# kai422/DAS3R

Hardware: AMD Instinct MI355X
Metric: render fwd+bwd Msplats/s at 1080p (higher is better)
Workload: dtype f32; 1 GPU; 1M random splats, 1920x1080, SH degree 3, forward+backward (BASELINE.json configs[3], constant P); splats_per_gpu=1000000, splats_per_gpu_final=1000000, init_steps=30, sh_degree=3, num_rendered=2614506, api=GaussianRasterizer.forward + autograd backward (drop-in surface), parallelism=1 independent scenes, one per GPU

## Files before the change

das3r_amd/csrc/api.hip:

```cpp
#include <stdarg.h>
#include <string.h>

#include <vector>

#include "common.h"
#include <algorithm>

namespace das3r {

static thread_local char g_err[512] = "";

void set_error(const char *fmt, ...) {
    va_list ap;
    va_start(ap, fmt);
    vsnprintf(g_err, sizeof(g_err), fmt, ap);
    va_end(ap);
}

struct ProfRec {
    const char *name;
    hipEvent_t start, stop;
};
static bool g_prof_on = false;
static std::vector<ProfRec> g_prof;
// ... 53 lines not shown
            const char *pp = strchr(e, 'p');
            w.render_bwd_pix = pp ? atoi(pp + 1) : 0;
            const char *po = strchr(e, 'o');
            w.render_bwd_occ = po ? atoi(po + 1) : 5;
        }
        if (w.render_bwd == 7) {
            const char *d = e;
            while (*d && (*d < '0' || *d > '9')) d++;
            w.render_bwd_mb = *d ? atoi(d) : 128;
            w.render_bwd_pix = strchr(e, 'q') ? 9 : (strchr(e, 's') ? 8 : 0);
        }
        if (w.render_bwd == 3) {
            const char *d = e;
            while (*d && (*d < '0' || *d > '9')) d++;
            w.render_bwd_mb = (*d ? atoi(d) : 256) + (strncmp(e, "scana", 5) == 0 ? 1000 : 0);
        }
    }
    if ((e = env("DAS3R_BWD_REDUCE"))) { w.bwd_reduce_set = true; w.bwd_reduce_shfl = e[0] == 's'; }
    w.tickets = -1;
    if ((e = env("DAS3R_TICKETS"))) w.tickets = e[0] == 'a' ? 0 : (e[0] == 'n' ? 1 << 30 : ((e[0] >= '1' && e[0] <= '9') ? atoi(e) : -1));
    w.deterministic = (e = env("DAS3R_DETERMINISTIC")) && e[0] != '0';
    w.bwd_buckets = -1;
    if ((e = env("DAS3R_BWD_BUCKETS"))) w.bwd_buckets = atoi(e);
    w.tile_strip = 8;
    w.tile_chunk = -1;
    if ((e = env("DAS3R_TILE_CHUNK"))) { const int v = atoi(e); w.tile_chunk = (v >= 0 && v <= 64 && (v & (v - 1)) == 0) ? v : -1; }
    if ((e = env("DAS3R_TILE_STRIP"))) w.tile_strip = std::max(0, std::min(63, atoi(e)));
    w.inject_fault = g_inject_fault;
    w.mutate = g_mutate;
    g_sw = w;
    __atomic_store_n(&g_sw_loaded, true, __ATOMIC_RELEASE);
}
const Switches &switches() {
    if (!__atomic_load_n(&g_sw_loaded, __ATOMIC_ACQUIRE)) load_switches();
    return g_sw;
}

constexpr int MAX_DEVICES = 64;
static int g_threads_on_device[MAX_DEVICES] = {};
struct ThreadRegistrar {
    bool on[MAX_DEVICES] = {};
    void add(int dev) {
        if (!on[dev]) { on[dev] = true; __atomic_fetch_add(&g_threads_on_device[dev], 1, __ATOMIC_RELAXED); }
    }
    ~ThreadRegistrar() {
        for (int d = 0; d < MAX_DEVICES; d++)
// ... 107 lines not shown
    L->g_dhist = take(4 * 256);
    L->g_ghist = take(4 * 4 * RADIX_SIZE);
    L->g_ticket = take(256);
    L->g_status = take(onesweep_status_bytes((int64_t)Pn, 4));
    L->g_scan_status = take(scan_status_bytes((int)Pn));
    L->g_ctrl_bytes = o - L->g_ghist;
    if (shjac) L->g_shjac = take(4 * 9 * Pn);
    L->pub.geom_bytes = o;
    o = 0;
    L->b_keyA = take(4 * In);
    L->b_keyB = take(4 * In);
    L->b_valA = take(4 * In);
    L->b_valB = take(4 * In);
    L->b_hist = take(4 * (size_t)RADIX_SIZE * (size_t)(L->chunksI > 0 ? L->chunksI : 1));
    L->b_totals = take(4 * RADIX_SIZE);
    L->b_gid_of = take(4 * In);
    L->b_slot = take(4 * In);
    L->b_e2 = take(4 * In);
    L->b_ghist = take(4 * 4 * RADIX_SIZE);
    L->b_ticket = take(256);
    L->b_status = take(onesweep_status_bytes((int64_t)In, L->tile_passes + 1));
    L->b_ctrl_bytes = o - L->b_ghist;
    L->b_ckpt = take(((size_t)In / BUCKET + (size_t)(L->ntiles > 0 ? L->ntiles : 1) + 2) * 256 * 16);
    L->pub.binning_bytes = o;
    const size_t npix_d = (size_t)W * (size_t)H;
    L->d_ckpt = take(((size_t)In / BUCKET + (size_t)(L->ntiles > 0 ? L->ntiles : 1) + 2) * 256 * 16);
    L->d_recs = take(16 * SPLAT_REC * Pn);
    L->d_dpix = take(4 * 3 * (npix_d > 0 ? npix_d : 1));
    L->d_bg = take(16);
    L->d_dz = take(4 * Pn);
    L->d_bytes = o;
    L->pub.point_list = (L->tile_passes & 1) ? L->b_valB : L->b_valA;
    o = 0;
    const size_t npix = (size_t)W * (size_t)H;
    L->pub.final_T = take(4 * (npix > 0 ? npix : 1));
    L->pub.n_contrib = take(4 * (npix > 0 ? npix : 1));
    L->pub.ranges = take(8 * (size_t)(L->ntiles > 0 ? L->ntiles : 1));
    L->i_order = take(4 * (size_t)(L->ntiles > 0 ? L->ntiles : 1));
    L->pub.img_bytes = o;
}

static bool dhist_slots(hipStream_t s, uint32_t **use, uint32_t **next) {
    struct Slot { int dev; hipStream_t stream; uint32_t *buf; uint32_t turn; };
    static thread_local std::vector<Slot> slots;
    int dev = 0;
    if (hipGetDevice(&dev) != hipSuccess) return false;
// ... 361 lines not shown
            verdict.longest = (uint32_t)longest;
            const uint32_t crowd16 = mb->host[15];
            verdict.fine = (longest > mean + (mean * 4) / 5 && longest >= 4096) || crowd16 >= CROWDED16;
            if (switches().verbose) fprintf(stderr, "[das3r] tile lists: longest %lld, mean %lld, %.1f of 64 consecutive entries in one quadrant -> %s kernels\n", (long long)longest,
                                            (long long)mean, crowd16 / 16.0, verdict.fine ? "2x2-region" : "block");
        }
        lb.prefer_regions = verdict.fine;
        lb.tile_order = nullptr;
        if (verdict.fine && cap > 0 && use_quad_lanes(L, lb) && L.ntiles <= 1024 && !switches().tile_lpt_off && (switches().render_fwd == 0 || switches().render_fwd == 5)) {
            if ((r = launch_tile_lpt(saved->img, L, (uint32_t)cap, a->debug != 0, s))) return r;
            lb.tile_order = (const uint32_t *)(saved->img + L.i_order);
        }
        if (verdict.fine && cap > 0 && use_quad_lanes(L, lb)) {
            const uint32_t hint = std::min<uint32_t>(63u, verdict.longest / (uint32_t)BUCKET + 2u);
            saved->flags |= 1u | (hint << 8);
        }
        if (local_order && cap > 0) {
            lb.point_list = (uint32_t *)(saved->binning + L.pub.point_list);
            lb.slot_list = (uint32_t *)(saved->binning + L.b_slot);
            lb.keys = dead_keys;
            lb.host_flag = mb->dev + 10;
        }
        if ((r = join.now())) return r;
        return launch_render_forward(a, in->colors_precomp, out->out_color, saved->geom, saved->binning, saved->img, L, lb, s, out->out_invdepth,
                                     depth ? (float4 *)(saved->binning + L.d_ckpt) : nullptr);
    };
    auto prefiltered_ok = [&]() -> int {
        if (!a->prefiltered || mb->host[12] != count_tag) return DAS3R_OK;
        set_error("Point is filtered although prefiltered is set. This shouldn't happen!");
        return DAS3R_ERR_INVALID_ARG;
    };
    int64_t I, cap;
    if ((local || seg) && verdict.last_I >= 0 && a->capacity_hint != -1 && !switches().capacity_exact) {
        cap = std::max(verdict.last_I + verdict.last_I / 4, verdict.peak_I + verdict.peak_I / 20) + 4096;
        if (cap > (int64_t)0x7FFFFF00) cap = (int64_t)0x7FFFFF00;
        compute_layout(P, cap, W, H, &L, shjac);
        apply_seg();
        saved->binning = alloc_binning(user, depth ? L.d_bytes : L.pub.binning_bytes);
        if (!saved->binning) { set_error("scratch allocation failed (binning %zu B)", L.pub.binning_bytes); return DAS3R_ERR_ALLOC; }
        char *&emit_ring = T->emit_ring;
        bool &emit_ring_dirty = T->emit_ring_dirty;
        uint32_t &emit_last_tag = T->emit_last_tag;
        constexpr size_t EMIT_SLOT_BYTES = sizeof(uint32_t) * EMIT_SLOT_WORDS + sizeof(unsigned long long) * EMIT_STATUS_GRANULES;
        const bool fused_emit = local && grid_is_resident(div_up(P, 256)) && !switches().fused_emit_off;
        uint32_t *emit_slot = nullptr;
        if (fused_emit) {
// ... 385 lines not shown
```

das3r_amd/csrc/common.h:

```cpp
#pragma once
#include <hip/hip_runtime.h>
#include <stdint.h>
#include <stdio.h>

#include "../../include/das3r_raster.h"
#include "pretransform_math.h"

#define TILE_X 16
#define TILE_Y 16
#define TILE_PIX 256
#define WAVE 64
#define NEAR_PLANE 0.001f

namespace das3r {

void set_error(const char *fmt, ...);

struct Switches {
    int sort_ipl;
    bool sort_classic;
    bool rect_upstream;
    bool verbose;
    int binning;
    bool capacity_exact;
    bool fused_emit_off;
    bool no_sh_stage;
    int render_fwd;
    int render_bwd;
    int render_bwd_mb;
    int tile_chunk;
    int scan_items;
    bool deterministic;
    int render_bwd_occ;
    bool tile_lpt_off;
    int render_bwd_pix;
    bool bwd_reduce_set, bwd_reduce_shfl;
    bool ablate_set;
    int ablate;
    int tickets;
    int bwd_pad_lds, fwd_pad_lds;
    int bwd_buckets;
    int inject_fault;
    int mutate;
    bool fwd_no_prefetch;
    int split_colour;
    int tile_strip;
};
const Switches &switches();

#define HIP_TRY(expr)                                                                          \
    do {                                                                                       \
        hipError_t _e = (expr);                                                                \
        if (_e != hipSuccess) {                                                                \
            das3r::set_error("%s failed: %s (%s:%d)", #expr, hipGetErrorString(_e), __FILE__, __LINE__); \
            return DAS3R_ERR_HIP;                                                              \
        }                                                                                      \
    } while (0)

#define KERNEL_CHECK(stream, debug, name)                                                      \
    do {                                                                                       \
        hipError_t _e = hipGetLastError();                                                     \
        if (_e == hipSuccess && (debug)) _e = hipStreamSynchronize(stream);                    \
        if (_e != hipSuccess) {                                                                \
            das3r::set_error("kernel %s failed: %s", name, hipGetErrorString(_e));             \
            return DAS3R_ERR_HIP;                                                              \
        }                                                                                      \
    } while (0)

// ... 77 lines not shown
int sort_ipl_override();
static inline int sort_items_per_lane(int64_t n) {
    const int o = sort_ipl_override();
    return o ? o : (n >= (int64_t)(1 << 21) ? 16 : (n >= (1 << 17) ? 8 : 4));
}
static inline int sort_num_chunks(int64_t n) { return n == 0 ? 0 : div_up(n, (int64_t)WAVE * sort_items_per_lane(n)); }
__host__ __device__ static inline int tile_digit_width(int tbits) {
    const int passes = (tbits + 7) / 8;
    return passes > 0 ? (tbits + passes - 1) / passes : 8;
}
static inline int tile_bits(int ntiles) {
    int b = 0;
    while ((1 << b) < ntiles) b++;
    return b < 1 ? 1 : b;
}

constexpr int BUCKET = 1024;
constexpr int SPLAT_REC = 4;

constexpr uint32_t DEPTH_SAVED_FLAG = 2u;
constexpr uint32_t SHJAC_SAVED_FLAG = 4u;
constexpr uint32_t NO_BACKWARD_IN_FLAG = 8u;
constexpr uint32_t ANTIALIAS_FLAG = 16u;
struct Layout {
    das3r_raster_layout pub;
    size_t g_keyA, g_keyB, g_valA, g_valB, g_hist, g_totals, g_blocksums, g_count, g_off_by_gid, g_rect;
    size_t b_keyA, b_keyB, b_valA, b_valB, b_hist, b_totals, b_gid_of, b_slot;
    size_t b_e2;
    size_t b_ckpt;
    size_t d_ckpt, d_recs, d_dpix, d_bg, d_dz, d_bytes;
    size_t g_ghist, g_ticket, g_status, g_scan_status, g_ctrl_bytes;
    int64_t capacity;
    size_t b_ghist, b_ticket, b_status, b_ctrl_bytes;
    int tiles_x, tiles_y, ntiles, tbits, tile_passes;
    int chunksP, chunksI;
    int dbits, kbits, kshift;
    int part_passes;
    size_t g_dhist;
    size_t g_shjac;
    const uint32_t *dhist_ptr;
    size_t i_order;
};
static inline int seg_dbits(const Layout &L, int passes) { return 8 * (passes < 3 ? passes : 3) - L.tbits; }

struct LocalBin {
    float4 *ckpt;
    uint32_t *point_list, *slot_list;
    uint32_t *keys;
    uint32_t *host_flag;
    uint32_t flag_value;
    uint32_t last_g, cap;
    bool prefer_regions;
// ... 19 lines not shown
struct SideStream {
    hipStream_t stream;
    hipEvent_t fork, join;
    int colour_blocks;
};
int launch_preprocess(const das3r_raster_args *a, const das3r_raster_in *in, int32_t *radii, char *geom, char *img, char *binning_ctrl,
                      size_t binning_ctrl_bytes, const Layout &L, unsigned long long *arrive, uint32_t *host_out, uint32_t tag,
                      hipStream_t s, const EmitArgs *emit, uint32_t *dhist, uint32_t *dhist_next, bool aa ,
                      const SideStream *side = nullptr);
int launch_sh_colour(const das3r_raster_args *a, const das3r_raster_in *in, char *geom, const Layout &L, const SideStream *side);
int launch_mark_visible(int P, const float *means3D, const float *viewmatrix, uint8_t *present, hipStream_t s);
int launch_depth_sort(int P, char *geom, const Layout &L, int part, char *binning_ctrl, size_t binning_ctrl_bytes, bool debug, hipStream_t s);
int launch_scan(int P, char *geom, const Layout &L, uint32_t *host_out, uint32_t tag, bool debug, hipStream_t s, bool index_order = false);
int launch_scan_emit(int P, int64_t cap, const int32_t *radii, char *geom, char *binning, const Layout &L, uint32_t *host_out, uint32_t tag,
                     bool debug, hipStream_t s, bool index_order = false);
size_t scan_status_bytes(int P);
int launch_binning_scan_emit(int P, int64_t I, const int32_t *radii, char *geom, char *binning, const Layout &L, bool ctrl_zeroed,
                             uint32_t *host_out, uint32_t tag, bool debug, hipStream_t s, bool index_order = false);
size_t onesweep_status_bytes(int64_t n, int passes);
int launch_onesweep_depth_sort(int P, char *geom, const Layout &L, int part, uint32_t *zero_ptr, uint32_t zero_words, bool debug,
                               hipStream_t s);
int launch_onesweep_partition(int64_t cap, char *geom, char *binning, const Layout &L, uint32_t **keys_final, bool debug, hipStream_t s,
                              uint32_t *ghist_override = nullptr, uint32_t *err_override = nullptr);
bool use_row_private(int64_t instances, int ntiles);
bool use_quad_lanes(const Layout &L, const LocalBin &lb);
inline PreXform pre_xform(const das3r_raster_in *in) {
    PreXform x = {nullptr, nullptr, nullptr, nullptr, nullptr, nullptr, nullptr, nullptr, nullptr};
    if (in && in->pre) {
        const das3r_pretransform *p = in->pre;
        x = PreXform{p->xyz, p->rot, p->scaling, p->opacity_raw, p->conf_flat, p->mask_index, p->R, p->t, p->Lq};
    }
    return x;
}
int launch_render_forward_regions(const das3r_raster_args *a, float *out_color, char *geom, char *binning, char *img, const Layout &L, const LocalBin &lb,
                                  hipStream_t s, float *out_invdepth, float4 *dckpt);
int launch_tile_lpt(char *img, const Layout &L, uint32_t cap, bool debug, hipStream_t s);
int launch_list_skew(const char *img, const char *binning, const char *geom, const Layout &L, uint32_t cap, uint32_t last_g, uint32_t *mailbox_words, uint32_t tag,
                     bool debug, hipStream_t s);
int launch_render_forward_slices(const das3r_raster_args *a, float *out_color, char *geom, char *binning, char *img, const Layout &L, const LocalBin &lb,
                                 hipStream_t s);
int launch_render_forward_lanes(const das3r_raster_args *a, float *out_color, char *geom, char *binning, char *img, const Layout &L,
                                const LocalBin &lb, hipStream_t s, float *out_invdepth, float4 *dckpt);
int launch_render_forward_rows(const das3r_raster_args *a, float *out_color, char *geom, char *binning, char *img, const Layout &L,
                               const LocalBin &lb, hipStream_t s, float *out_invdepth, float4 *dckpt);
int launch_render_backward_mfma(const das3r_raster_args *a, const float *dL_dpix, char *geom, char *binning, char *img, const Layout &L,
                                float *partial, hipStream_t s);
size_t stream_scratch_bytes(int64_t capacity);
int launch_render_backward_stream(const das3r_raster_args *a, const float *dL_dpix, char *geom, char *binning, char *img, const Layout &L,
                                  float *scratch, hipStream_t s);
int launch_render_backward_scan(const das3r_raster_args *a, const float *dL_dpix, char *geom, char *binning, char *img, const Layout &L,
                                float *partial, int mb, int slices, hipStream_t s);
int launch_render_backward_blk(const das3r_raster_args *a, const float *dL_dpix, char *geom, char *binning, char *img, const Layout &L,
                               float *partial, int mb, int slices, hipStream_t s);
int launch_render_backward_regions(const das3r_raster_args *a, const float *dL_dpix, char *geom, char *binning, char *img, const Layout &L,
                               float *partial, int mb, int slices, hipStream_t s);
constexpr int LOCAL_MAX = 1024;
bool grid_is_resident(int nblocks);
bool use_onesweep();
bool use_tight_rect();
int launch_binning(int P, int64_t I, int W, int H, const int32_t *radii, char *geom, char *binning, char *img, const Layout &L,
                   bool fused_scan, uint32_t *host_late, uint32_t tag, bool debug, hipStream_t s, uint32_t **dead_keys = nullptr,
                   uint32_t *emit_slot = nullptr ,
                   uint32_t *seg_host_flag = nullptr, uint32_t seg_flag_value = 0 );
int launch_segment_sort(int64_t cap, const uint32_t *n_ptr, const uint32_t *keys_final, int fbits, uint32_t *point_list, uint32_t *slot_list,
                        const uint32_t *depth_key, uint32_t last_g, uint32_t *scratch_keys, uint32_t *host_flag, uint32_t flag_value, bool debug,
                        hipStream_t s, int dbits, uint2 *ranges, const uint32_t *err, uint32_t *host_late, uint32_t tag, uint32_t inject);
int launch_render_forward(const das3r_raster_args *a, const float *colors_precomp, float *out_color, char *geom, char *binning,
                          char *img, const Layout &L, const LocalBin &lb, hipStream_t s, float *out_invdepth ,
                          float4 *dckpt );
int launch_depth_pass_inputs(int P, int npix, const char *geom, const Layout &L, char *binning, const float *dL_dinvdepth, hipStream_t s, bool debug);
int launch_depth_fold(int P, const char *geom, const Layout &L, float *partial, const float *partial_depth, float *dz, hipStream_t s, bool debug);
int launch_render_backward(const das3r_raster_args *a, const float *dL_dpix, char *geom, char *binning, char *img, const Layout &L,
                           float *partial, hipStream_t s, bool *quad_rows, int64_t num_rendered, uint32_t fwd_flags );
int launch_render_aux_forward(int P, int W, int H, int C, const float *feat, float *out, const char *geom, const char *binning, const char *img,
                              const Layout &L, int64_t num_rendered, bool debug, hipStream_t s);
int launch_render_aux_adjoint(int P, int W, int H, int C, const float *dL_dout, float *dL_dfeat, int accumulate, float *partial, const char *geom,
// ... 39 lines not shown
```

das3r_amd/csrc/render_bwd.hip:

```cpp
#include "render_common.h"

namespace das3r {

constexpr int NACC = 9;

template <bool USE_DPP>
__global__ void __launch_bounds__(256) render_backward_kernel(
    const uint2 *__restrict__ ranges, const uint32_t *__restrict__ point_list, int W, int H, int tiles_x, int ntiles_strip ,
    const float4 *__restrict__ xyh, const float4 *__restrict__ conic_opacity, const float4 *__restrict__ rgbd,
    const float *__restrict__ bg, const float *__restrict__ final_T, const uint32_t *__restrict__ n_contrib,
    const float *__restrict__ dL_dpix, const uint32_t *__restrict__ slot_list, float *__restrict__ partial , int ablate,
    uint32_t last_g, uint32_t cap ,
    unsigned long long *__restrict__ pairs ) {
    __shared__ StagedSplat stage[TILE_PIX];
    __shared__ uint32_t s_slot[TILE_PIX];
    __shared__ float acc[TILE_PIX * NACC];
    __shared__ uint32_t s_max[4];

    const int ntiles = packed_ntiles(ntiles_strip);
    const int tile = xcd_tile(blockIdx.x, ntiles_strip, tiles_x);
    if (tile < 0) return;
    const int tid = threadIdx.x, lane = __lane_id(), wave = tid >> 6;
    const int bx = tile % tiles_x, by = tile / tiles_x;
    int px, py;
// ... 131 lines not shown
        if (sw.deterministic && kind == 1) {
            kind = 6;
            mb = 64;
        }
    }
#ifdef DAS3R_EXPERIMENTS
    if (kind == 5) {
        *quad_rows = true;
        return launch_render_backward_stream(a, dL_dpix, geom, binning, img, L, partial, s);
    }
    if (kind == 2) return launch_render_backward_mfma(a, dL_dpix, geom, binning, img, L, partial, s);
#else
    if (kind == 5 || kind == 2) {
        set_error("DAS3R_RENDER_BWD=%s: this library was built without the superseded kernels (make EXPERIMENTS=1)", kind == 5 ? "stream" : "mfma");
        return DAS3R_ERR_INVALID_ARG;
    }
#endif
    if (kind == 3 || kind == 6 || kind == 7) {
        int slices = sw.bwd_buckets;
        if (slices < 0) slices = (int)std::min<int64_t>(32, std::max<int64_t>(1, num_rendered / ((int64_t)BUCKET * std::max(L.ntiles, 1))));
        if (slices > 1 && mb > 256) slices = 1;
        const int hint = (int)((fwd_flags >> 8) & 0xFFu);
        if (sw.bwd_buckets < 0 && kind == 7 && slices > 1 && hint > slices) slices = std::min(hint, 64);
        if (kind == 6) return launch_render_backward_blk(a, dL_dpix, geom, binning, img, L, partial, mb, slices, s);
        if (kind == 7) return launch_render_backward_regions(a, dL_dpix, geom, binning, img, L, partial, mb, slices, s);
        return launch_render_backward_scan(a, dL_dpix, geom, binning, img, L, partial, mb, slices, s);
    }
    const bool use_dpp = !sw.bwd_reduce_shfl;
    const int ablate = sw.ablate;
#define ARGS                                                                                                                 \
    (const uint2 *)(img + L.pub.ranges), (const uint32_t *)(binning + L.pub.point_list), a->image_width, a->image_height,    \
        L.tiles_x, pack_tiles(L), (const float4 *)(geom + L.pub.xy), (const float4 *)(geom + L.pub.conic_opacity),                \
        (const float4 *)(geom + L.pub.rgbd), a->bg, (const float *)(img + L.pub.final_T),                                    \
        (const uint32_t *)(img + L.pub.n_contrib), dL_dpix, (const uint32_t *)(binning + L.b_slot), partial, ablate, \
        (uint32_t)(a->P - 1), (uint32_t)L.capacity, pair_counters()
    const int pad_lds = sw.bwd_pad_lds;
    if (use_dpp) DAS3R_LAUNCH((render_backward_kernel<true>), dim3(xcd_grid(L)), dim3(TILE_PIX), pad_lds, s, ARGS);
    else DAS3R_LAUNCH((render_backward_kernel<false>), dim3(xcd_grid(L)), dim3(TILE_PIX), 0, s, ARGS);
#undef ARGS
    KERNEL_CHECK(s, a->debug, "render_backward");
    return DAS3R_OK;
}

}
```

das3r_amd/csrc/render_bwd_blk.hip:

```cpp
#include "render_blk.h"

namespace das3r {

template <int MB, int PIX, int ABL = 0, int OCC = 5, bool LAST = false>
__global__ void __launch_bounds__(256, OCC) render_backward_blk_kernel(
    const uint2 *__restrict__ ranges, const uint32_t *__restrict__ point_list, int W, int H, int tiles_x, int ntiles_strip ,
    const float4 *__restrict__ xyh, const float4 *__restrict__ conic_opacity, const float4 *__restrict__ rgbd,
    const float *__restrict__ bg, const float *__restrict__ final_T, const uint32_t *__restrict__ n_contrib,
    const float *__restrict__ dL_dpix, const uint32_t *__restrict__ slot_list, float *__restrict__ partial ,
    uint32_t last_g, uint32_t cap ,
    const float4 *__restrict__ ckpt ,
    unsigned long long *__restrict__ pairs_arg ) {
#ifdef DAS3R_EXPERIMENTS
    DECODE_PAIRS_OR_TRACE(pairs_arg)
#else
    unsigned long long *const pairs = pairs_arg;
#endif
    static_assert(MB >= 64 && MB <= 256 && MB % 8 == 0, "entries per round (one-byte list entries)");
    constexpr int LIST_STRIDE = MB + 4;
    constexpr int OFF_STAGE = 0;
    constexpr int OFF_ACC = OFF_STAGE + MB * (int)sizeof(StagedSplat);
    constexpr int OFF_ACC1 = OFF_ACC + 4 * MB * 8 * 4;
    constexpr int OFF_SLOT = OFF_ACC1 + 4 * MB * 4;
    constexpr int OFF_LIST = OFF_SLOT + MB * 4;
    constexpr int OFF_MAX = OFF_LIST + 16 * LIST_STRIDE;
    constexpr int OFF_CST = OFF_MAX + 16;
    constexpr int OFF_ST = OFF_CST + (PIX > 0 ? 16 * PIX_CST_ROW : 0);
    constexpr int LDS_BYTES = OFF_ST + (PIX == 2 ? 16 * PIX_ST_ROW : 0);
    __shared__ __attribute__((aligned(16))) char lds[LDS_BYTES];
    StagedSplat *const stage = reinterpret_cast<StagedSplat *>(lds + OFF_STAGE);
    float *const acc8 = reinterpret_cast<float *>(lds + OFF_ACC);
    float *const acc1 = reinterpret_cast<float *>(lds + OFF_ACC1);
    uint32_t *const s_slot = reinterpret_cast<uint32_t *>(lds + OFF_SLOT);
    uint32_t *const s_max = reinterpret_cast<uint32_t *>(lds + OFF_MAX);

// ... 66 lines not shown
            for (uint32_t f = tid; f < ntail; f += TILE_PIX) {
                const uint32_t t = f / NACC, q = f - t * NACC;
                partial[(size_t)min(slot_list[range.x + lo + max_contrib + t], cap - 1u) * NACC + q] = 0.f;
            }
        }
        PHASE_MARK(14)
        if (max_contrib == 0u) continue;
        if (slices > 1) {
            float T0 = my_T_final, R0 = 0.f;
            if (bk < nbuckets - 1) {
                const int cpix = (ppy - by * TILE_Y) * 16 + (ppx - bx * TILE_X);
                const float4 far = ckpt_slot(const_cast<float4 *>(ckpt), range, tile, bk)[cpix];
                const float4 fin = ckpt_slot(const_cast<float4 *>(ckpt), range, tile, nbuckets - 1)[cpix];
                T0 = far.x;
                R0 = px.d0 * (fin.y - far.y) + px.d1 * (fin.z - far.z) + px.d2 * (fin.w - far.w);
            }
            px.T = T0;
            px.R = R0 + my_tfbg;
            if constexpr (PIX == 2) {
                *reinterpret_cast<float2 *>(st_row + s * 8) = make_float2(px.T, px.R);
                __builtin_amdgcn_fence(__ATOMIC_ACQ_REL, "workgroup");
            }
        }
        uint32_t g_ahead = 0u, slot_ahead = 0u;
        if (tid < min(MB, (int)max_contrib)) {
            const uint32_t pos = range.x + lo + max_contrib - 1 - tid;
            g_ahead = point_list[pos];
            slot_ahead = slot_list[pos];
        }
        for (int i = 0; i < rounds; i++) {
            const int done_before = i * MB;
            const int n = min(MB, (int)max_contrib - done_before);
            if (tid < n) {
                const uint32_t g = min(g_ahead, last_g);
                s_slot[tid] = min(slot_ahead, cap - 1u);
                stage[tid].xyh = xyh[(size_t)g * SPLAT_REC];
                stage[tid].co = conic_opacity[(size_t)g * SPLAT_REC];
                stage[tid].rgbd = rgbd[(size_t)g * SPLAT_REC];
            }
            if (i + 1 < rounds && tid < min(MB, (int)max_contrib - done_before - MB)) {
                const uint32_t pos = range.x + lo + max_contrib - 1 - (done_before + MB) - tid;
                g_ahead = point_list[pos];
                slot_ahead = slot_list[pos];
            }
            {
                const long long base = (long long)lo + (long long)max_contrib - done_before - MB;
                const long long rel = (long long)last_contributor - base;
                px.lastrel = (float)(rel < 0 ? 0ll : (rel > MB ? (long long)MB : rel));
                if constexpr (PIX > 0) *reinterpret_cast<float *>(cst_row + s * 16 + 12) = px.lastrel;
            }
            float blk_last[4] = {0.f, 0.f, 0.f, 0.f};
            if constexpr (LAST) {
                int v = (int)px.lastrel;
#pragma unroll
                for (int o = 8; o >= 1; o >>= 1) v = max(v, __shfl_xor(v, o, 64));
#pragma unroll
                for (int r = 0; r < 4; r++) blk_last[r] = (float)__builtin_amdgcn_readlane(v, 16 * r);
            }
            __syncthreads();
            PHASE_MARK(9)

            int len[4] = {0, 0, 0, 0};
#pragma unroll
            for (int k = 0; k < (MB + 63) / 64; k++) {
                const int j = k * 64 + lane;
                const int jc = j < n ? j : 0;
                const float4 p = stage[jc].xyh;
                const float4 co = stage[jc].co;
                const bool qhit = (j < n) && ((ABL & 16) ? rect_hit_tight_tau(p, co, splat_tau(co.w), (float)qx0, (float)qy0) : true);
                float hd1, hd2;
                diagonal_extents(p, co, hd1, hd2);
                const float posrel_j = (float)(MB - 1 - j);
#pragma unroll
                for (int r = 0; r < 4; r++) {
                    const bool hit = qhit && (!LAST || posrel_j < blk_last[r]) && block_hit_oct(p.x, p.y, p.z, p.w, (ABL & 8) ? 1e30f : hd1, (ABL & 8) ? 1e30f : hd2,
                                                           (float)(qx0 + ((r & 1) << 2)) + 1.5f, (float)(qy0 + ((r >> 1) << 2)) + 1.5f);
                    const uint64_t m = __ballot(hit);
                    const int at = len[r] + (int)__builtin_amdgcn_mbcnt_hi((uint32_t)(m >> 32), __builtin_amdgcn_mbcnt_lo((uint32_t)m, 0u));
                    if (hit) wave_lists[r * LIST_STRIDE + at] = (uint8_t)j;
                    len[r] += __popcll(m);
                }
            }
            const int my_len = row == 0 ? len[0] : (row == 1 ? len[1] : (row == 2 ? len[2] : len[3]));
            const int longest = (ABL & 1) ? 0 : __builtin_amdgcn_readfirstlane(max(max(len[0], len[1]), max(len[2], len[3])));
            __builtin_amdgcn_fence(__ATOMIC_ACQ_REL, "workgroup");
            PHASE_MARK(10)

            v4f p_lo4 = {0.f, 0.f, 0.f, 0.f}, p_hi4 = p_lo4;
            float p_syy = 0.f;
            float *p_rec8 = acc8, *p_rec1 = acc1;
            bool p_valid = false;
            auto add_pass = [&](const int r) {
                if (row == r && p_valid && !(ABL & 2)) {
                    const v4f o0 = *reinterpret_cast<const v4f *>(p_rec8), o1 = *reinterpret_cast<const v4f *>(p_rec8 + 4 * MB * 4);
                    const float o2 = *p_rec1;
                    *reinterpret_cast<v4f *>(p_rec8) = o0 + p_lo4;
                    *reinterpret_cast<v4f *>(p_rec8 + 4 * MB * 4) = o1 + p_hi4;
                    *p_rec1 = o2 + p_syy;
                }
                __builtin_amdgcn_fence(__ATOMIC_ACQ_REL, "wavefront");
            };
            batches_done += (longest + 15) >> 4;
            for (int b = 0; b < longest; b += 16) {
// ... 59 lines not shown
                    store_partial_row(rowp, a[0], a[1], a[2], (Sgx * co.x + Sgy * co.y) * (float)W ,
                                      (Sgy * co.z + Sgx * co.y) * (float)H, kh * a[6], kh * a[7], kh * a[8], a[3]);
                }
            }
            PHASE_MARK(13)
        }
    }
    PHASE_END(8)
#ifdef DAS3R_EXPERIMENTS
    BLK_STAMP(trace, 5, 1)
    if (trace != nullptr) {
        asm volatile("s_waitcnt vmcnt(0)" ::: "memory");
        BLK_STAMP(trace, 5, 2)
        if (threadIdx.x == 0 && blockIdx.x < (uint32_t)TRACE_WGS) trace[((size_t)5 * TRACE_WGS + blockIdx.x) * TRACE_STAMPS + 3] = range.y - range.x;
    }
#endif
    if (pairs != nullptr && lane == 0 && batches_done > 0) {
        atomicAdd(pairs + 1, (unsigned long long)batches_done * 1024ull);
        atomicAdd(pairs + 3, (unsigned long long)batches_done * 16ull);
    }
}

int launch_render_backward_blk(const das3r_raster_args *a, const float *dL_dpix, char *geom, char *binning, char *img, const Layout &L,
                               float *partial, int mb, int slices, hipStream_t s) {
#define ARGS                                                                                                              \
    (const uint2 *)(img + L.pub.ranges), (const uint32_t *)(binning + L.pub.point_list), a->image_width, a->image_height, \
        L.tiles_x, pack_tiles(L), (const float4 *)(geom + L.pub.xy), (const float4 *)(geom + L.pub.conic_opacity),             \
        (const float4 *)(geom + L.pub.rgbd), a->bg, (const float *)(img + L.pub.final_T),                                 \
        (const uint32_t *)(img + L.pub.n_contrib), dL_dpix, (const uint32_t *)(binning + L.b_slot), partial,              \
        (uint32_t)(a->P - 1), (uint32_t)L.capacity, (const float4 *)(binning + L.b_ckpt), PAIRS_ARG
#define GO(MBV, PIX, OCC)                                                                                                                             \
    do {                                                                                                                                              \
        if (slices > 1) DAS3R_LAUNCH((render_backward_blk_kernel<MBV, PIX, 0, OCC, true>), dim3(xcd_grid(L), slices), dim3(TILE_PIX), 0, s, ARGS);   \
        else DAS3R_LAUNCH((render_backward_blk_kernel<MBV, PIX, 0, OCC, false>), dim3(xcd_grid(L), 1), dim3(TILE_PIX), 0, s, ARGS);                   \
    } while (0)
    const int pix = switches().render_bwd == 6 ? switches().render_bwd_pix : (mb == 128 ? 1 : 0), occ = switches().render_bwd_occ == 4 ? 4 : 5;
#define BY_PIX(MBV, OCC) do { if (pix == 2) GO(MBV, 2, OCC); else if (pix == 1) GO(MBV, 1, OCC); else GO(MBV, 0, OCC); } while (0)
    if (switches().mutate == 1) {
        if (slices > 1) DAS3R_LAUNCH((render_backward_blk_kernel<192, 0, 32, 4, true>), dim3(xcd_grid(L), slices), dim3(TILE_PIX), 0, s, ARGS);
        else DAS3R_LAUNCH((render_backward_blk_kernel<128, 1, 32, 5, false>), dim3(xcd_grid(L), 1), dim3(TILE_PIX), 0, s, ARGS);
    } else
#ifdef DAS3R_EXPERIMENTS
    if (mb == 128 && pix == 1 && switches().ablate_set) {
        const int abl = switches().ablate;
#define GA(A) DAS3R_LAUNCH((render_backward_blk_kernel<128, 1, A>), dim3(xcd_grid(L), slices > 1 ? slices : 1), dim3(TILE_PIX), 0, s, ARGS)
        if (abl == 1) GA(1); else if (abl == 2) GA(2); else if (abl == 4) GA(4); else if (abl == 8) GA(8); else if (abl == 16) GA(16); else if (abl == 3) GA(3); else if (abl == 7) GA(7); else GA(0);
#undef GA
    } else
#endif
    if (mb == 64) BY_PIX(64, 5);
    else if (mb == 256) BY_PIX(256, 5);
    else if (mb == 120) BY_PIX(120, 5);
    else if (mb == 160) BY_PIX(160, 4);
    else if (mb == 192) BY_PIX(192, 4);
    else if (occ == 4) BY_PIX(128, 4);
    else BY_PIX(128, 5);
#undef BY_PIX
#undef GO
#undef ARGS
    KERNEL_CHECK(s, a->debug, "render_backward_blk");
    return DAS3R_OK;
}

}
```

das3r_amd/csrc/render_rows.hip:

```cpp
#include "render_common.h"

namespace das3r {

__device__ __forceinline__ void block_pixel(const int bx, const int by, const int wave, const int lane, int &px, int &py) {
    const int row = lane >> 4;
    px = bx * TILE_X + ((wave & 1) << 3) + ((row & 1) << 2) + (lane & 3);
    py = by * TILE_Y + ((wave >> 1) << 3) + ((row >> 1) << 2) + ((lane >> 2) & 3);
}

__device__ __forceinline__ bool block_hit(const float4 xyh, const float cx, const float cy) {
    return fabsf(xyh.x - cx) <= xyh.z + 1.5f && fabsf(xyh.y - cy) <= xyh.w + 1.5f;
}

constexpr int ROW_LIST_STRIDE = TILE_PIX;

template <bool OCT>
__device__ __forceinline__ void build_row_lists(const StagedSplat *stage, const int n, const float q0x, const float q0y, const int lane,
                                                uint8_t (*lists)[ROW_LIST_STRIDE], int len[4]) {
    len[0] = len[1] = len[2] = len[3] = 0;
#pragma unroll
    for (int k = 0; k < 4; k++) {
        const int s = k * 64 + lane;
        const bool valid = s < n;
        const float4 p = stage[valid ? s : 0].xyh;
        float hd1 = 1e30f, hd2 = 1e30f;
        if constexpr (OCT) diagonal_extents(p, stage[valid ? s : 0].co, hd1, hd2);
#pragma unroll
        for (int r = 0; r < 4; r++) {
            const float bcx = q0x + (float)((r & 1) << 2) + 1.5f, bcy = q0y + (float)((r >> 1) << 2) + 1.5f;
            const bool hit = valid && (OCT ? block_hit_oct(p.x, p.y, p.z, p.w, hd1, hd2, bcx, bcy) : block_hit(p, bcx, bcy));
            const uint64_t m = __ballot(hit);
            const int pos = len[r] + (int)__builtin_amdgcn_mbcnt_hi((uint32_t)(m >> 32), __builtin_amdgcn_mbcnt_lo((uint32_t)m, 0u));
            if (hit) lists[r][pos] = (uint8_t)s;
            len[r] += __popcll(m);
        }
    }
}

#define FWD_WAVES(PREFETCH) __attribute__((amdgpu_waves_per_eu((PREFETCH) ? 1 : 8, 8)))
template <bool PREFETCH, bool DEPTH = false>
__global__ void __launch_bounds__(256) FWD_WAVES(PREFETCH || DEPTH) render_forward_rows_kernel(const uint2 *__restrict__ ranges, const uint32_t *__restrict__ point_list,
                                                                  int W, int H, int tiles_x, int ntiles_strip , const float4 *__restrict__ xyh,
                                                                  const float4 *__restrict__ conic_opacity,
                                                                  const float4 *__restrict__ rgbd, const float *__restrict__ bg,
                                                                  float *__restrict__ final_T, uint32_t *__restrict__ n_contrib,
                                                                  float *__restrict__ out_color, const LocalBin lb,
                                                                  unsigned long long *__restrict__ pairs_arg ,
                                                                  float *__restrict__ out_invdepth, float4 *__restrict__ dckpt) {
#ifdef DAS3R_EXPERIMENTS
    DECODE_PAIRS_OR_TRACE(pairs_arg)
#else
    unsigned long long *const pairs = pairs_arg;
#endif
    constexpr int NBUF = PREFETCH ? 2 : 1;
    __shared__ StagedSplat stage_all[NBUF * TILE_PIX];
    StagedSplat *stage = stage_all;
    __shared__ uint32_t s_gid[LOCAL_MAX];
    __shared__ uint8_t lists[4][4][ROW_LIST_STRIDE];
    const int ntiles = packed_ntiles(ntiles_strip);
    const int tile = xcd_tile(blockIdx.x, ntiles_strip, tiles_x);
    if (tile < 0) return;
    PHASE_BEGIN();
#ifdef DAS3R_EXPERIMENTS
    BLK_STAMP(trace, 4, 0)
#endif
    const int tid = threadIdx.x, lane = __lane_id(), wave = tid >> 6, row = lane >> 4;
    const int bx = tile % tiles_x, by = tile / tiles_x;
    int px, py;
    block_pixel(bx, by, wave, lane, px, py);
    const bool inside = px < W && py < H;
    const float pxf = (float)px, pyf = (float)py;
// ... 54 lines not shown
            }
            if (progress + TILE_PIX < range.y) {
                const uint32_t g = min(g_ahead, lb.last_g);
                pf0 = xyh[(size_t)g * SPLAT_REC];
                pf1 = conic_opacity[(size_t)g * SPLAT_REC];
                pf2 = rgbd[(size_t)g * SPLAT_REC];
            }
            if (progress + 2 * TILE_PIX < range.y) g_ahead = point_list[progress + 2 * TILE_PIX];
        } else if (progress < range.y && !prestaged) {
            const uint32_t g = min(sorted_here ? s_gid[i * TILE_PIX + tid] : (lb.point_list ? lb.point_list[progress] : point_list[progress]), lb.last_g);
            stage[tid].xyh = xyh[(size_t)g * SPLAT_REC];
            stage[tid].co = conic_opacity[(size_t)g * SPLAT_REC];
            if constexpr (DEPTH) stage[tid].rgbd = staged_invz(rgbd[(size_t)g * SPLAT_REC]);
            else stage[tid].rgbd = rgbd[(size_t)g * SPLAT_REC];
        } else if (!prestaged) {
            stage[tid] = null_splat();
        }
        if (PREFETCH) lds_barrier();
        else __syncthreads();
        const int n = toDo < TILE_PIX ? toDo : TILE_PIX;
        PHASE_MARK(2)
        int len[4];
        blend_batch_begin(pb);
        build_row_lists<!PREFETCH>(stage, n, q0x, q0y, lane, lists[wave], len);
        const int my_len = row == 0 ? len[0] : (row == 1 ? len[1] : (row == 2 ? len[2] : len[3]));
        const int longest = max(max(len[0], len[1]), max(len[2], len[3]));
        const uint8_t *mine = lists[wave][row];
        PHASE_MARK(3)
        constexpr int UNROLL = 4;
        const float lenf = (float)my_len;
        for (int t = 0; t < longest; t += UNROLL) {
            if ((t & 15) == 0 && __ballot(live != 0.f) == 0ull) break;
            positions += UNROLL;
            int jj[UNROLL];
            float aa[UNROLL];
            const float rem = lenf - (float)t;
            const uint32_t packed = *reinterpret_cast<const uint32_t *>(mine + t);
#pragma unroll
            for (int u = 0; u < UNROLL; u++) {
                const int j = (int)((packed >> (8 * u)) & 0xFFu);
                const float4 p = stage[j].xyh;
                const float4 co = stage[j].co;
                const float dx = p.x - pxf, dy = p.y - pyf;
                const float q = __fmaf_rn(__fmul_rn(co.x, dx), dx, __fmul_rn(__fmul_rn(co.z, dy), dy));
                const float power = __fmaf_rn(-0.5f, q, -__fmul_rn(__fmul_rn(co.y, dx), dy));
                const float a1 = fminf(fminf(0.99f, __fmul_rn(co.w, __expf(power))), rem - (float)u);
                jj[u] = j;
// ... 24 lines not shown
    }
    PHASE_MARK(5)
    PHASE_END(0)
#ifdef DAS3R_EXPERIMENTS
    BLK_STAMP(trace, 4, 1)
    if (trace != nullptr) {
        asm volatile("s_waitcnt vmcnt(0)" ::: "memory");
        BLK_STAMP(trace, 4, 2)
        if (threadIdx.x == 0 && blockIdx.x < (uint32_t)TRACE_WGS) trace[((size_t)4 * TRACE_WGS + blockIdx.x) * TRACE_STAMPS + 3] = range.y - range.x;
    }
#endif
    if (pairs != nullptr && lane == 0 && positions > 0) {
        atomicAdd(pairs, (unsigned long long)positions * 64ull);
        atomicAdd(pairs + 2, (unsigned long long)positions);
    }
}

bool use_row_private(int64_t instances, int ntiles) {
    const int forced = switches().render_fwd;
    if (forced == 1 || forced == 2) return forced == 2;
    return instances >= (int64_t)128 * ntiles;
}

int launch_render_forward_rows(const das3r_raster_args *a, float *out_color, char *geom, char *binning, char *img, const Layout &L,
                               const LocalBin &lb, hipStream_t s, float *out_invdepth, float4 *dckpt) {
#define ARGS                                                                                                              \
    (const uint2 *)(img + L.pub.ranges), (const uint32_t *)(binning + L.pub.point_list), a->image_width, a->image_height,  \
        L.tiles_x, pack_tiles(L), (const float4 *)(geom + L.pub.xy), (const float4 *)(geom + L.pub.conic_opacity),         \
        (const float4 *)(geom + L.pub.rgbd), a->bg, (float *)(img + L.pub.final_T), (uint32_t *)(img + L.pub.n_contrib),   \
        out_color, lb, PAIRS_ARG, out_invdepth, dckpt
    const bool prefetch = lb.point_list == nullptr && L.ntiles <= 1024 && !switches().fwd_no_prefetch;
    if (out_invdepth) {
        if (prefetch) DAS3R_LAUNCH((render_forward_rows_kernel<true, true>), dim3(xcd_grid(L)), dim3(TILE_PIX), 0, s, ARGS);
        else DAS3R_LAUNCH((render_forward_rows_kernel<false, true>), dim3(xcd_grid(L)), dim3(TILE_PIX), 0, s, ARGS);
    } else if (prefetch) DAS3R_LAUNCH((render_forward_rows_kernel<true>), dim3(xcd_grid(L)), dim3(TILE_PIX), 0, s, ARGS);
    else DAS3R_LAUNCH((render_forward_rows_kernel<false>), dim3(xcd_grid(L)), dim3(TILE_PIX), 0, s, ARGS);
#undef ARGS
    KERNEL_CHECK(s, a->debug, "render_forward_rows");
    return DAS3R_OK;
}

}
```

Baseline: 1196 Msplats/s.

## Reuse forward per-block hit masks in backward blk kernel to skip culling

The rows forward kernel now writes a per-splat-instance byte mask recording which 4x4 sub-blocks each splat hits, stored in a new binning buffer. When the forward path leaves these masks, the backward blk kernel loads them alongside the point list and builds its per-row lists from the bits instead of recomputing diagonal extents and octagon hit tests. This trades the backward geometry culling for an extra 4-byte-per-instance write in forward and a read in backward, and it only applies to a few MB/PIX/occupancy combinations and non-prefetch forward paths.

```diff
diff --git a/das3r_amd/csrc/api.hip b/das3r_amd/csrc/api.hip
--- a/das3r_amd/csrc/api.hip
+++ b/das3r_amd/csrc/api.hip
@@ -99,6 +99,7 @@
     w.deterministic = (e = env("DAS3R_DETERMINISTIC")) && e[0] != '0';
     w.bwd_buckets = -1;
     if ((e = env("DAS3R_BWD_BUCKETS"))) w.bwd_buckets = atoi(e);
+    if ((e = env("DAS3R_BWD_CULL"))) w.bwd_cull = e[0] == 'o' ? 1 : 0;
     w.tile_strip = 8;
     w.tile_chunk = -1;
     if ((e = env("DAS3R_TILE_CHUNK"))) { const int v = atoi(e); w.tile_chunk = (v >= 0 && v <= 64 && (v & (v - 1)) == 0) ? v : -1; }
@@ -252,6 +253,7 @@
     L->b_status = take(onesweep_status_bytes((int64_t)In, L->tile_passes + 1));
     L->b_ctrl_bytes = o - L->b_ghist;
     L->b_ckpt = take(((size_t)In / BUCKET + (size_t)(L->ntiles > 0 ? L->ntiles : 1) + 2) * 256 * 16);
+    L->b_mask = take(4 * In);
     L->pub.binning_bytes = o;
     const size_t npix_d = (size_t)W * (size_t)H;
     L->d_ckpt = take(((size_t)In / BUCKET + (size_t)(L->ntiles > 0 ? L->ntiles : 1) + 2) * 256 * 16);
@@ -659,6 +661,7 @@
             lb.host_flag = mb->dev + 10;
         }
         if ((r = join.now())) return r;
+        saved->flags = (saved->flags & ~BLOCK_MASKS_FLAG) | (cap > 0 && rows_forward_leaves_masks(L, lb) ? BLOCK_MASKS_FLAG : 0u);
         return launch_render_forward(a, in->colors_precomp, out->out_color, saved->geom, saved->binning, saved->img, L, lb, s, out->out_invdepth,
                                      depth ? (float4 *)(saved->binning + L.d_ckpt) : nullptr);
     };
diff --git a/das3r_amd/csrc/common.h b/das3r_amd/csrc/common.h
--- a/das3r_amd/csrc/common.h
+++ b/das3r_amd/csrc/common.h
@@ -44,6 +44,7 @@
     int mutate;
     bool fwd_no_prefetch;
     int split_colour;
+    int bwd_cull;
     int tile_strip;
 };
 const Switches &switches();
@@ -167,12 +168,14 @@
 constexpr uint32_t SHJAC_SAVED_FLAG = 4u;
 constexpr uint32_t NO_BACKWARD_IN_FLAG = 8u;
 constexpr uint32_t ANTIALIAS_FLAG = 16u;
+constexpr uint32_t BLOCK_MASKS_FLAG = 32u;
 struct Layout {
     das3r_raster_layout pub;
     size_t g_keyA, g_keyB, g_valA, g_valB, g_hist, g_totals, g_blocksums, g_count, g_off_by_gid, g_rect;
     size_t b_keyA, b_keyB, b_valA, b_valB, b_hist, b_totals, b_gid_of, b_slot;
     size_t b_e2;
     size_t b_ckpt;
+    size_t b_mask;
     size_t d_ckpt, d_recs, d_dpix, d_bg, d_dz, d_bytes;
     size_t g_ghist, g_ticket, g_status, g_scan_status, g_ctrl_bytes;
     int64_t capacity;
@@ -238,6 +241,7 @@
                                hipStream_t s);
 int launch_onesweep_partition(int64_t cap, char *geom, char *binning, const Layout &L, uint32_t **keys_final, bool debug, hipStream_t s,
                               uint32_t *ghist_override = nullptr, uint32_t *err_override = nullptr);
+bool rows_forward_leaves_masks(const Layout &L, const LocalBin &lb);
 bool use_row_private(int64_t instances, int ntiles);
 bool use_quad_lanes(const Layout &L, const LocalBin &lb);
 inline PreXform pre_xform(const das3r_raster_in *in) {
@@ -267,7 +271,7 @@
 int launch_render_backward_scan(const das3r_raster_args *a, const float *dL_dpix, char *geom, char *binning, char *img, const Layout &L,
                                 float *partial, int mb, int slices, hipStream_t s);
 int launch_render_backward_blk(const das3r_raster_args *a, const float *dL_dpix, char *geom, char *binning, char *img, const Layout &L,
-                               float *partial, int mb, int slices, hipStream_t s);
+                               float *partial, int mb, int slices, hipStream_t s, uint32_t fwd_flags );
 int launch_render_backward_regions(const das3r_raster_args *a, const float *dL_dpix, char *geom, char *binning, char *img, const Layout &L,
                                float *partial, int mb, int slices, hipStream_t s);
 constexpr int LOCAL_MAX = 1024;
diff --git a/das3r_amd/csrc/render_bwd.hip b/das3r_amd/csrc/render_bwd.hip
--- a/das3r_amd/csrc/render_bwd.hip
+++ b/das3r_amd/csrc/render_bwd.hip
@@ -177,7 +177,7 @@
         if (slices > 1 && mb > 256) slices = 1;
         const int hint = (int)((fwd_flags >> 8) & 0xFFu);
         if (sw.bwd_buckets < 0 && kind == 7 && slices > 1 && hint > slices) slices = std::min(hint, 64);
-        if (kind == 6) return launch_render_backward_blk(a, dL_dpix, geom, binning, img, L, partial, mb, slices, s);
+        if (kind == 6) return launch_render_backward_blk(a, dL_dpix, geom, binning, img, L, partial, mb, slices, s, fwd_flags);
         if (kind == 7) return launch_render_backward_regions(a, dL_dpix, geom, binning, img, L, partial, mb, slices, s);
         return launch_render_backward_scan(a, dL_dpix, geom, binning, img, L, partial, mb, slices, s);
     }
diff --git a/das3r_amd/csrc/render_bwd_blk.hip b/das3r_amd/csrc/render_bwd_blk.hip
--- a/das3r_amd/csrc/render_bwd_blk.hip
+++ b/das3r_amd/csrc/render_bwd_blk.hip
@@ -2,7 +2,7 @@
 
 namespace das3r {
 
-template <int MB, int PIX, int ABL = 0, int OCC = 5, bool LAST = false>
+template <int MB, int PIX, int ABL = 0, int OCC = 5, bool LAST = false, bool REUSE = false>
 __global__ void __launch_bounds__(256, OCC) render_backward_blk_kernel(
     const uint2 *__restrict__ ranges, const uint32_t *__restrict__ point_list, int W, int H, int tiles_x, int ntiles_strip ,
     const float4 *__restrict__ xyh, const float4 *__restrict__ conic_opacity, const float4 *__restrict__ rgbd,
@@ -10,7 +10,8 @@
     const float *__restrict__ dL_dpix, const uint32_t *__restrict__ slot_list, float *__restrict__ partial ,
     uint32_t last_g, uint32_t cap ,
     const float4 *__restrict__ ckpt ,
-    unsigned long long *__restrict__ pairs_arg ) {
+    unsigned long long *__restrict__ pairs_arg ,
+    const uint32_t *__restrict__ masks ) {
 #ifdef DAS3R_EXPERIMENTS
     DECODE_PAIRS_OR_TRACE(pairs_arg)
 #else
@@ -123,11 +124,12 @@
                 __builtin_amdgcn_fence(__ATOMIC_ACQ_REL, "workgroup");
             }
         }
-        uint32_t g_ahead = 0u, slot_ahead = 0u;
+        uint32_t g_ahead = 0u, slot_ahead = 0u, mask_ahead = 0u;
         if (tid < min(MB, (int)max_contrib)) {
             const uint32_t pos = range.x + lo + max_contrib - 1 - tid;
             g_ahead = point_list[pos];
             slot_ahead = slot_list[pos];
+            if constexpr (REUSE) mask_ahead = masks[pos];
         }
         for (int i = 0; i < rounds; i++) {
             const int done_before = i * MB;
@@ -138,11 +140,13 @@
                 stage[tid].xyh = xyh[(size_t)g * SPLAT_REC];
                 stage[tid].co = conic_opacity[(size_t)g * SPLAT_REC];
                 stage[tid].rgbd = rgbd[(size_t)g * SPLAT_REC];
+                if constexpr (REUSE) stage[tid].rgbd.w = __uint_as_float(mask_ahead);
             }
             if (i + 1 < rounds && tid < min(MB, (int)max_contrib - done_before - MB)) {
                 const uint32_t pos = range.x + lo + max_contrib - 1 - (done_before + MB) - tid;
                 g_ahead = point_list[pos];
                 slot_ahead = slot_list[pos];
+                if constexpr (REUSE) mask_ahead = masks[pos];
             }
             {
                 const long long base = (long long)lo + (long long)max_contrib - done_before - MB;
@@ -162,24 +166,41 @@
             PHASE_MARK(9)
 
             int len[4] = {0, 0, 0, 0};
-#pragma unroll
-            for (int k = 0; k < (MB + 63) / 64; k++) {
-                const int j = k * 64 + lane;
-                const int jc = j < n ? j : 0;
-                const float4 p = stage[jc].xyh;
-                const float4 co = stage[jc].co;
-                const bool qhit = (j < n) && ((ABL & 16) ? rect_hit_tight_tau(p, co, splat_tau(co.w), (float)qx0, (float)qy0) : true);
-                float hd1, hd2;
-                diagonal_extents(p, co, hd1, hd2);
-                const float posrel_j = (float)(MB - 1 - j);
-#pragma unroll
-                for (int r = 0; r < 4; r++) {
-                    const bool hit = qhit && (!LAST || posrel_j < blk_last[r]) && block_hit_oct(p.x, p.y, p.z, p.w, (ABL & 8) ? 1e30f : hd1, (ABL & 8) ? 1e30f : hd2,
-                                                           (float)(qx0 + ((r & 1) << 2)) + 1.5f, (float)(qy0 + ((r >> 1) << 2)) + 1.5f);
-                    const uint64_t m = __ballot(hit);
-                    const int at = len[r] + (int)__builtin_amdgcn_mbcnt_hi((uint32_t)(m >> 32), __builtin_amdgcn_mbcnt_lo((uint32_t)m, 0u));
-                    if (hit) wave_lists[r * LIST_STRIDE + at] = (uint8_t)j;
-                    len[r] += __popcll(m);
+            if constexpr (REUSE) {
+#pragma unroll
+                for (int k = 0; k < (MB + 63) / 64; k++) {
+                    const int j = k * 64 + lane;
+                    const uint32_t bits = j < n ? (__float_as_uint(stage[j < n ? j : 0].rgbd.w) >> (8 * wave)) & 0xFu : 0u;
+                    const float posrel_j = (float)(MB - 1 - j);
+#pragma unroll
+                    for (int r = 0; r < 4; r++) {
+                        const bool hit = ((bits >> r) & 1u) != 0u && (!LAST || posrel_j < blk_last[r]);
+                        const uint64_t m = __ballot(hit);
+                        const int at = len[r] + (int)__builtin_amdgcn_mbcnt_hi((uint32_t)(m >> 32), __builtin_amdgcn_mbcnt_lo((uint32_t)m, 0u));
+                        if (hit) wave_lists[r * LIST_STRIDE + at] = (uint8_t)j;
+                        len[r] += __popcll(m);
+                    }
+                }
+            } else {
+    #pragma unroll
+                for (int k = 0; k < (MB + 63) / 64; k++) {
+                    const int j = k * 64 + lane;
+                    const int jc = j < n ? j : 0;
+                    const float4 p = stage[jc].xyh;
+                    const float4 co = stage[jc].co;
+                    const bool qhit = (j < n) && ((ABL & 16) ? rect_hit_tight_tau(p, co, splat_tau(co.w), (float)qx0, (float)qy0) : true);
+                    float hd1, hd2;
+                    diagonal_extents(p, co, hd1, hd2);
+                    const float posrel_j = (float)(MB - 1 - j);
+    #pragma unroll
+                    for (int r = 0; r < 4; r++) {
+                        const bool hit = qhit && (!LAST || posrel_j < blk_last[r]) && block_hit_oct(p.x, p.y, p.z, p.w, (ABL & 8) ? 1e30f : hd1, (ABL & 8) ? 1e30f : hd2,
+                                                               (float)(qx0 + ((r & 1) << 2)) + 1.5f, (float)(qy0 + ((r >> 1) << 2)) + 1.5f);
+                        const uint64_t m = __ballot(hit);
+                        const int at = len[r] + (int)__builtin_amdgcn_mbcnt_hi((uint32_t)(m >> 32), __builtin_amdgcn_mbcnt_lo((uint32_t)m, 0u));
+                        if (hit) wave_lists[r * LIST_STRIDE + at] = (uint8_t)j;
+                        len[r] += __popcll(m);
+                    }
                 }
             }
             const int my_len = row == 0 ? len[0] : (row == 1 ? len[1] : (row == 2 ? len[2] : len[3]));
@@ -285,19 +306,26 @@
 }
 
 int launch_render_backward_blk(const das3r_raster_args *a, const float *dL_dpix, char *geom, char *binning, char *img, const Layout &L,
-                               float *partial, int mb, int slices, hipStream_t s) {
+                               float *partial, int mb, int slices, hipStream_t s, uint32_t fwd_flags) {
 #define ARGS                                                                                                              \
     (const uint2 *)(img + L.pub.ranges), (const uint32_t *)(binning + L.pub.point_list), a->image_width, a->image_height, \
         L.tiles_x, pack_tiles(L), (const float4 *)(geom + L.pub.xy), (const float4 *)(geom + L.pub.conic_opacity),             \
         (const float4 *)(geom + L.pub.rgbd), a->bg, (const float *)(img + L.pub.final_T),                                 \
         (const uint32_t *)(img + L.pub.n_contrib), dL_dpix, (const uint32_t *)(binning + L.b_slot), partial,              \
-        (uint32_t)(a->P - 1), (uint32_t)L.capacity, (const float4 *)(binning + L.b_ckpt), PAIRS_ARG
+        (uint32_t)(a->P - 1), (uint32_t)L.capacity, (const float4 *)(binning + L.b_ckpt), PAIRS_ARG, (const uint32_t *)(binning + L.b_mask)
 #define GO(MBV, PIX, OCC)                                                                                                                             \
     do {                                                                                                                                              \
         if (slices > 1) DAS3R_LAUNCH((render_backward_blk_kernel<MBV, PIX, 0, OCC, true>), dim3(xcd_grid(L), slices), dim3(TILE_PIX), 0, s, ARGS);   \
         else DAS3R_LAUNCH((render_backward_blk_kernel<MBV, PIX, 0, OCC, false>), dim3(xcd_grid(L), 1), dim3(TILE_PIX), 0, s, ARGS);                   \
     } while (0)
     const int pix = switches().render_bwd == 6 ? switches().render_bwd_pix : (mb == 128 ? 1 : 0), occ = switches().render_bwd_occ == 4 ? 4 : 5;
+    const bool reuse = (fwd_flags & BLOCK_MASKS_FLAG) != 0 && switches().bwd_cull != 1;
+#define GO4(MBV, PIX, OCC, LASTV)                                                                                                                     \
+    do {                                                                                                                                              \
+        const dim3 grid(xcd_grid(L), (LASTV) ? slices : 1);                                                                                           \
+        if (reuse) DAS3R_LAUNCH((render_backward_blk_kernel<MBV, PIX, 0, OCC, LASTV, true>), grid, dim3(TILE_PIX), 0, s, ARGS);                       \
+        else DAS3R_LAUNCH((render_backward_blk_kernel<MBV, PIX, 0, OCC, LASTV, false>), grid, dim3(TILE_PIX), 0, s, ARGS);                            \
+    } while (0)
 #define BY_PIX(MBV, OCC) do { if (pix == 2) GO(MBV, 2, OCC); else if (pix == 1) GO(MBV, 1, OCC); else GO(MBV, 0, OCC); } while (0)
     if (switches().mutate == 1) {
         if (slices > 1) DAS3R_LAUNCH((render_backward_blk_kernel<192, 0, 32, 4, true>), dim3(xcd_grid(L), slices), dim3(TILE_PIX), 0, s, ARGS);
@@ -311,7 +339,10 @@
 #undef GA
     } else
 #endif
-    if (mb == 64) BY_PIX(64, 5);
+    if (mb == 128 && pix == 1 && occ == 5) { if (slices > 1) GO4(128, 1, 5, true); else GO4(128, 1, 5, false); }
+    else if (mb == 128 && pix == 1) { if (slices > 1) GO4(128, 1, 4, true); else GO4(128, 1, 4, false); }
+    else if (mb == 192 && pix == 0) { if (slices > 1) GO4(192, 0, 4, true); else GO4(192, 0, 4, false); }
+    else if (mb == 64) BY_PIX(64, 5);
     else if (mb == 256) BY_PIX(256, 5);
     else if (mb == 120) BY_PIX(120, 5);
     else if (mb == 160) BY_PIX(160, 4);
@@ -319,6 +350,7 @@
     else if (occ == 4) BY_PIX(128, 4);
     else BY_PIX(128, 5);
 #undef BY_PIX
+#undef GO4
 #undef GO
 #undef ARGS
     KERNEL_CHECK(s, a->debug, "render_backward_blk");
diff --git a/das3r_amd/csrc/render_rows.hip b/das3r_amd/csrc/render_rows.hip
--- a/das3r_amd/csrc/render_rows.hip
+++ b/das3r_amd/csrc/render_rows.hip
@@ -16,7 +16,7 @@
 
 template <bool OCT>
 __device__ __forceinline__ void build_row_lists(const StagedSplat *stage, const int n, const float q0x, const float q0y, const int lane,
-                                                uint8_t (*lists)[ROW_LIST_STRIDE], int len[4]) {
+                                                uint8_t (*lists)[ROW_LIST_STRIDE], int len[4], uint8_t *mask_bytes = nullptr) {
     len[0] = len[1] = len[2] = len[3] = 0;
 #pragma unroll
     for (int k = 0; k < 4; k++) {
@@ -25,6 +25,7 @@
         const float4 p = stage[valid ? s : 0].xyh;
         float hd1 = 1e30f, hd2 = 1e30f;
         if constexpr (OCT) diagonal_extents(p, stage[valid ? s : 0].co, hd1, hd2);
+        uint32_t bits = 0u;
 #pragma unroll
         for (int r = 0; r < 4; r++) {
             const float bcx = q0x + (float)((r & 1) << 2) + 1.5f, bcy = q0y + (float)((r >> 1) << 2) + 1.5f;
@@ -33,7 +34,10 @@
             const int pos = len[r] + (int)__builtin_amdgcn_mbcnt_hi((uint32_t)(m >> 32), __builtin_amdgcn_mbcnt_lo((uint32_t)m, 0u));
             if (hit) lists[r][pos] = (uint8_t)s;
             len[r] += __popcll(m);
-        }
+            bits |= (hit ? 1u : 0u) << r;
+        }
+        if constexpr (OCT)
+            if (mask_bytes != nullptr && valid) mask_bytes[256 * k + 4 * lane] = (uint8_t)bits;
     }
 }
 
@@ -46,7 +50,8 @@
                                                                   float *__restrict__ final_T, uint32_t *__restrict__ n_contrib,
                                                                   float *__restrict__ out_color, const LocalBin lb,
                                                                   unsigned long long *__restrict__ pairs_arg ,
-                                                                  float *__restrict__ out_invdepth, float4 *__restrict__ dckpt) {
+                                                                  float *__restrict__ out_invdepth, float4 *__restrict__ dckpt,
+                                                                  uint8_t *__restrict__ masks ) {
 #ifdef DAS3R_EXPERIMENTS
     DECODE_PAIRS_OR_TRACE(pairs_arg)
 #else
@@ -147,7 +152,8 @@
         PHASE_MARK(2)
         int len[4];
         blend_batch_begin(pb);
-        build_row_lists<!PREFETCH>(stage, n, q0x, q0y, lane, lists[wave], len);
+        build_row_lists<!PREFETCH>(stage, n, q0x, q0y, lane, lists[wave], len,
+                                   PREFETCH ? nullptr : masks + ((size_t)range.x + (size_t)i * TILE_PIX) * 4 + __builtin_amdgcn_readfirstlane(wave));
         const int my_len = row == 0 ? len[0] : (row == 1 ? len[1] : (row == 2 ? len[2] : len[3]));
         const int longest = max(max(len[0], len[1]), max(len[2], len[3]));
         const uint8_t *mine = lists[wave][row];
@@ -218,14 +224,19 @@
     return instances >= (int64_t)128 * ntiles;
 }
 
+static bool rows_prefetch(const Layout &L, const LocalBin &lb) { return lb.point_list == nullptr && L.ntiles <= 1024 && !switches().fwd_no_prefetch; }
+bool rows_forward_leaves_masks(const Layout &L, const LocalBin &lb) {
+    return !use_quad_lanes(L, lb) && use_row_private(L.capacity, L.ntiles) && !rows_prefetch(L, lb);
+}
+
 int launch_render_forward_rows(const das3r_raster_args *a, float *out_color, char *geom, char *binning, char *img, const Layout &L,
                                const LocalBin &lb, hipStream_t s, float *out_invdepth, float4 *dckpt) {
 #define ARGS                                                                                                              \
     (const uint2 *)(img + L.pub.ranges), (const uint32_t *)(binning + L.pub.point_list), a->image_width, a->image_height,  \
         L.tiles_x, pack_tiles(L), (const float4 *)(geom + L.pub.xy), (const float4 *)(geom + L.pub.conic_opacity),         \
         (const float4 *)(geom + L.pub.rgbd), a->bg, (float *)(img + L.pub.final_T), (uint32_t *)(img + L.pub.n_contrib),   \
-        out_color, lb, PAIRS_ARG, out_invdepth, dckpt
-    const bool prefetch = lb.point_list == nullptr && L.ntiles <= 1024 && !switches().fwd_no_prefetch;
+        out_color, lb, PAIRS_ARG, out_invdepth, dckpt, (uint8_t *)(binning + L.b_mask)
+    const bool prefetch = rows_prefetch(L, lb);
     if (out_invdepth) {
         if (prefetch) DAS3R_LAUNCH((render_forward_rows_kernel<true, true>), dim3(xcd_grid(L)), dim3(TILE_PIX), 0, s, ARGS);
         else DAS3R_LAUNCH((render_forward_rows_kernel<false, true>), dim3(xcd_grid(L)), dim3(TILE_PIX), 0, s, ARGS);
```

Measured after the change: 1216 Msplats/s, median of 6. 1.6% higher.
